# zhaotudou/HeteroFusionRCNN

Measured on AMD Instinct MI355X. Metric: KITTI frames/sec RPN train step, higher is better.
Workload: dtype f32; 1 GPU; RPN train step, hf/configs/rpn_multiclass.config: PointCNN 5 xconv (K=8; 16384/4096/1024/256/64 points; C 256..1024, X-transformation, global branch) + 6 xdconv layers + fc 256/256, 3 classes, seg head, projection of the points into the image + gather of the image feature map (B,360,1200,32) + path drop 0.9/0.9 + 'concat' fusion, bin-based box head (fc 512/512, 3x76 outputs), targets + focal/softm; frames_per_gpu=8, global_batch=8, parallelism=dp1, hip_graph=True, optimizer=hf, x_branch_on_side_stream=True, scaling=strong, library_gemm_selection=library default heuristic, gradient_exchange=none (1 rank), geometry_prefetch_depth=2, geometry_prefetch_group=12

## Files before the change

### heterofusionrcnn_amd/csrc/xconv.hip

```cpp
#include "hf_common.h"

namespace hf {

template <int M>
__device__ __forceinline__ void store_m(float *base, size_t elem, const float (&v)[M])
{
    float *p = base + elem;
    if constexpr (M == 4 || M == 8) {
        if ((reinterpret_cast<uintptr_t>(base) & 15) == 0) {
#pragma unroll
            for (int q = 0; q < M / 4; ++q) reinterpret_cast<float4 *>(p)[q] = make_float4(v[4 * q], v[4 * q + 1], v[4 * q + 2], v[4 * q + 3]);
            return;
        }
    } else if constexpr (M == 2) {
        if ((reinterpret_cast<uintptr_t>(base) & 7) == 0) { *reinterpret_cast<float2 *>(p) = make_float2(v[0], v[1]); return; }
    }
#pragma unroll
    for (int m = 0; m < M; ++m) p[m] = v[m];
}
template <int M>
__device__ __forceinline__ void load_m(const float *base, size_t elem, float (&v)[M])
{
    const float *p = base + elem;
    if constexpr (M == 4 || M == 8) {
        if ((reinterpret_cast<uintptr_t>(base) & 15) == 0) {
#pragma unroll
            for (int q = 0; q < M / 4; ++q) {
                const float4 t = reinterpret_cast<const float4 *>(p)[q];
                v[4 * q] = t.x; v[4 * q + 1] = t.y; v[4 * q + 2] = t.z; v[4 * q + 3] = t.w;
            }
            return;
        }
    } else if constexpr (M == 2) {
        if ((reinterpret_cast<uintptr_t>(base) & 7) == 0) { const float2 t = *reinterpret_cast<const float2 *>(p); v[0] = t.x; v[1] = t.y; return; }
    }
#pragma unroll
    for (int m = 0; m < M; ++m) v[m] = p[m];
}


constexpr int kXcThreads = 256;

template <int K, bool TRANSPOSED>
__global__ __launch_bounds__(kXcThreads) void xconv_apply_kernel(long long rows, int c, const float *__restrict__ x,
                                                                const float *__restrict__ f, float *__restrict__ out)
{
    const int lane = threadIdx.x & 63;
    const long long wave = __builtin_amdgcn_readfirstlane(static_cast<int>(threadIdx.x >> 6)) +
                           static_cast<long long>(blockIdx.x) * (kXcThreads / 64);
    const long long nwaves = static_cast<long long>(gridDim.x) * (kXcThreads / 64);
    for (long long r = wave; r < rows; r += nwaves) {
        const float *xr = x + r * (K * K);
        float coef[K][K];
#pragma unroll
        for (int i = 0; i < K; ++i)
#pragma unroll
            for (int j = 0; j < K; ++j) coef[i][j] = TRANSPOSED ? xr[j * K + i] : xr[i * K + j];
        const float *fr = f + r * K * c;
        float *orow = out + r * K * c;
        for (int ch = lane; ch < c; ch += 64) {
            float v[K];
#pragma unroll
            for (int j = 0; j < K; ++j) v[j] = fr[static_cast<size_t>(j) * c + ch];
#pragma unroll
            for (int i = 0; i < K; ++i) {
                float acc = coef[i][0] * v[0];
#pragma unroll
                for (int j = 1; j < K; ++j) acc = acc + coef[i][j] * v[j];
                orow[static_cast<size_t>(i) * c + ch] = acc;
            }
        }
    }
}

template <int K>
__global__ __launch_bounds__(kXcThreads) void xconv_dx_kernel(long long rows, int c, const float *__restrict__ grad_out,
                                                             const float *__restrict__ f, float *__restrict__ grad_x)
{
    extern __shared__ float lds[];
    constexpr int KK = K * K, STRIDE = KK + 1;
    const int lane = threadIdx.x & 63, w = threadIdx.x >> 6;
    float *mine = lds + static_cast<size_t>(w) * 64 * STRIDE;
    const long long wave = w + static_cast<long long>(blockIdx.x) * (kXcThreads / 64);
    const long long nwaves = static_cast<long long>(gridDim.x) * (kXcThreads / 64);
    for (long long r = wave; r < rows; r += nwaves) {
        const float *gr = grad_out + r * K * c;
        const float *fr = f + r * K * c;
        float acc[K][K];
#pragma unroll
        for (int i = 0; i < K; ++i)
#pragma unroll
            for (int j = 0; j < K; ++j) acc[i][j] = 0.f;
        for (int ch = lane; ch < c; ch += 64) {
            float g[K], v[K];
#pragma unroll
            for (int j = 0; j < K; ++j) { g[j] = gr[static_cast<size_t>(j) * c + ch]; v[j] = fr[static_cast<size_t>(j) * c + ch]; }
#pragma unroll
            for (int i = 0; i < K; ++i)
#pragma unroll
                for (int j = 0; j < K; ++j) acc[i][j] = acc[i][j] + g[i] * v[j];
        }
#pragma unroll
        for (int i = 0; i < K; ++i)
#pragma unroll
            for (int j = 0; j < K; ++j) mine[lane * STRIDE + i * K + j] = acc[i][j];
        __builtin_amdgcn_fence(__ATOMIC_SEQ_CST, "wavefront");
        __builtin_amdgcn_wave_barrier();
        for (int p = lane; p < KK; p += 64) {
            float s = 0.f;
            for (int l = 0; l < 64; ++l) s = s + mine[l * STRIDE + p];
            grad_x[r * KK + p] = s;
        }
        __builtin_amdgcn_fence(__ATOMIC_SEQ_CST, "wavefront");
        __builtin_amdgcn_wave_barrier();
    }
}

template <int K, int M>
__global__ __launch_bounds__(kXcThreads) void depthwise_fwd_kernel(long long rows, int c, const float *__restrict__ x,
                                                                  const float *__restrict__ wgt, float *__restrict__ y)
{
    const long long total = rows * c;
    for (long long g = static_cast<long long>(blockIdx.x) * kXcThreads + threadIdx.x; g < total;
         g += static_cast<long long>(gridDim.x) * kXcThreads) {
        const long long r = g / c;
        const int ch = static_cast<int>(g - r * c);
        float acc[M];
#pragma unroll
        for (int m = 0; m < M; ++m) acc[m] = 0.f;
#pragma unroll
        for (int w = 0; w < K; ++w) {
            const float xv = x[(r * K + w) * c + ch];
#pragma unroll
            for (int m = 0; m < M; ++m) acc[m] = acc[m] + xv * wgt[(static_cast<size_t>(w) * c + ch) * M + m];
        }
        store_m<M>(y, static_cast<size_t>(g) * M, acc);
    }
}

template <int K, int M>
__global__ __launch_bounds__(kXcThreads) void depthwise_dx_kernel(long long rows, int c, const float *__restrict__ grad_y,
                                                                 const float *__restrict__ wgt, float *__restrict__ grad_x)
{
    const long long total = rows * c;
    for (long long g = static_cast<long long>(blockIdx.x) * kXcThreads + threadIdx.x; g < total;
         g += static_cast<long long>(gridDim.x) * kXcThreads) {
        const long long r = g / c;
        const int ch = static_cast<int>(g - r * c);
        float gy[M];
        load_m<M>(grad_y, static_cast<size_t>(g) * M, gy);
#pragma unroll
        for (int w = 0; w < K; ++w) {
            float acc = 0.f;
#pragma unroll
            for (int m = 0; m < M; ++m) acc = acc + gy[m] * wgt[(static_cast<size_t>(w) * c + ch) * M + m];
            grad_x[(r * K + w) * c + ch] = acc;
        }
    }
}

template <int K, int M, bool DX>
__global__ __launch_bounds__(kXcThreads) void depthwise_narrow_kernel(long long rows, int c, const float *__restrict__ in,
                                                                     const float *__restrict__ wgt, float *__restrict__ out)
{
    const long long tid = static_cast<long long>(blockIdx.x) * kXcThreads + threadIdx.x;
    const long long nthreads = static_cast<long long>(gridDim.x) * kXcThreads;
    const int ch = static_cast<int>(tid % c);
    float wr[K][M];
#pragma unroll
    for (int w = 0; w < K; ++w)
#pragma unroll
        for (int m = 0; m < M; ++m) wr[w][m] = wgt[(static_cast<size_t>(w) * c + ch) * M + m];
    for (long long r = tid / c; r < rows; r += nthreads / c) {
        if (!DX) {
            float acc[M];
#pragma unroll
            for (int m = 0; m < M; ++m) acc[m] = 0.f;
#pragma unroll
            for (int w = 0; w < K; ++w) {
                const float xv = in[(r * K + w) * c + ch];
#pragma unroll
                for (int m = 0; m < M; ++m) acc[m] = acc[m] + xv * wr[w][m];
            }
            store_m<M>(out, static_cast<size_t>(r * c + ch) * M, acc);
        } else {
            float gy[M];
            load_m<M>(in, static_cast<size_t>(r * c + ch) * M, gy);
#pragma unroll
            for (int w = 0; w < K; ++w) {
                float acc = 0.f;
#pragma unroll
                for (int m = 0; m < M; ++m) acc = acc + gy[m] * wr[w][m];
                out[(r * K + w) * c + ch] = acc;
            }
        }
    }
}

static int narrow_grid(long long rows, int c)
{
    int a = c, b = kXcThreads;
    while (b) { const int tmp = a % b; a = b; b = tmp; }
    const int unit = c / a;
    long long g = (rows * c + kXcThreads - 1) / kXcThreads;
    const long long cap = static_cast<long long>(kNumCU) * 8;
    if (g > cap) g = cap;
    g = (g + unit - 1) / unit * unit;
    return static_cast<int>(g);
}
constexpr int kNarrowMaxC = 64;

template <int K, int M>
__global__ __launch_bounds__(kXcThreads) void depthwise_dw_kernel(long long rows, int c, int rows_per_chunk,
                                                                 const float *__restrict__ x, const float *__restrict__ grad_y,
                                                                 float *__restrict__ grad_w, float *__restrict__ partial)
{
    extern __shared__ float red[];
    const int cw = c < kXcThreads ? c : kXcThreads, nrs = kXcThreads / cw;
    const int t = static_cast<int>(threadIdx.x);
    const int cl = t % cw, ch = blockIdx.x * cw + cl, rs = t / cw;
    const bool live = ch < c && rs < nrs;
    if (nrs > 1) {
        for (int i = t; i < K * M * cw; i += kXcThreads) red[i] = 0.f;
        __syncthreads();
    }
    const long long r0 = static_cast<long long>(blockIdx.y) * rows_per_chunk + rs;
    const long long r1 = static_cast<long long>(blockIdx.y + 1) * rows_per_chunk < rows ? static_cast<long long>(blockIdx.y + 1) * rows_per_chunk : rows;
    float acc[K][M];
#pragma unroll
    for (int w = 0; w < K; ++w)
#pragma unroll
        for (int m = 0; m < M; ++m) acc[w][m] = 0.f;
    if (live) {
        for (long long r = r0; r < r1; r += nrs) {
            float gy[M];
            load_m<M>(grad_y, static_cast<size_t>(r * c + ch) * M, gy);
#pragma unroll
            for (int w = 0; w < K; ++w) {
                const float xv = x[(r * K + w) * c + ch];
#pragma unroll
                for (int m = 0; m < M; ++m) acc[w][m] = acc[w][m] + xv * gy[m];
            }
        }
    }
    float *mine = partial ? partial + static_cast<size_t>(blockIdx.y) * K * c * M : nullptr;
    if (nrs == 1) {
        if (live) {
#pragma unroll
            for (int w = 0; w < K; ++w)
#pragma unroll
                for (int m = 0; m < M; ++m) {
                    const size_t e = (static_cast<size_t>(w) * c + ch) * M + m;
                    if (mine) mine[e] = acc[w][m];
                    else atomicAdd(&grad_w[e], acc[w][m]);
                }
        }
        return;
    }
    const bool shuffle = (cw & (cw - 1)) == 0 && cw <= 32;
    if (shuffle) {
        const int lane = t & 63, wave = t >> 6;
        __syncthreads();
#pragma unroll
        for (int w = 0; w < K; ++w)
#pragma unroll
            for (int m = 0; m < M; ++m) {
                float v = live ? acc[w][m] : 0.f;
                for (int off = cw; off < 64; off <<= 1) v += __shfl_xor(v, off);
                if (lane < cw) red[(wave * K * M + w * M + m) * cw + lane] = v;
            }
        __syncthreads();
        for (int i = t; i < K * M * cw; i += kXcThreads) {
            float v = red[i];
#pragma unroll
            for (int wv = 1; wv < kXcThreads / 64; ++wv) v += red[wv * K * M * cw + i];
            const int wm = i / cw, c2 = blockIdx.x * cw + i % cw;
            if (c2 < c) {
                const size_t e = (static_cast<size_t>(wm / M) * c + c2) * M + wm % M;
                if (mine) mine[e] = v;
                else atomicAdd(&grad_w[e], v);
            }
        }
        return;
    }
    if (live) {
#pragma unroll
        for (int w = 0; w < K; ++w)
#pragma unroll
            for (int m = 0; m < M; ++m) atomicAdd(&red[(w * M + m) * cw + cl], acc[w][m]);
    }
    __syncthreads();
    for (int i = t; i < K * M * cw; i += kXcThreads) {
        const int wm = i / cw, c2 = blockIdx.x * cw + i % cw;
        if (c2 < c) {
            const size_t e = (static_cast<size_t>(wm / M) * c + c2) * M + wm % M;
            if (mine) mine[e] = red[i];
            else atomicAdd(&grad_w[e], red[i]);
        }
    }
}

struct XcSource {
    const float *base;
    long long stride;
    bool gathered;
};

__device__ __forceinline__ XcSource xc_source(int ch, int c, int c0, const float *f, const float *fts, const int *idx)
{
    XcSource s;
    if (idx == nullptr) { s.base = f + ch; s.stride = c; s.gathered = false; }
    else if (ch - (ch & 63) < c0) { s.base = f + ch; s.stride = c0; s.gathered = false; }
    else { s.base = fts + (ch - c0); s.stride = c - c0; s.gathered = true; }
    return s;
}

template <int K, int M, bool GATHER>
__global__ __launch_bounds__(kXcThreads) void xconv_dw_fwd_kernel(long long rows, int c, int c0, int rows_per_block,
                                                                 const float *__restrict__ x, const float *__restrict__ f,
                                                                 const float *__restrict__ fts, const int *__restrict__ idx, int n_src,
                                                                 int rows_per_cloud, const float *__restrict__ wd, float *__restrict__ out)
{
    const int lane = threadIdx.x & 63, wave = __builtin_amdgcn_readfirstlane(static_cast<int>(threadIdx.x >> 6));
    const int ch = blockIdx.y * 64 + lane;
    const bool live = ch < c;
    const XcSource src = xc_source(live ? ch : blockIdx.y * 64, c, c0, f, fts, GATHER ? idx : nullptr);
    float w[K][M];
#pragma unroll
    for (int k = 0; k < K; ++k)
#pragma unroll
        for (int m = 0; m < M; ++m) w[k][m] = live ? wd[(static_cast<size_t>(k) * c + ch) * M + m] : 0.f;
    const long long r0 = static_cast<long long>(blockIdx.x) * rows_per_block;
    const long long r1 = r0 + rows_per_block < rows ? r0 + rows_per_block : rows;
    for (long long r = r0 + wave; r < r1; r += kXcThreads / 64) {
        const float *xr = x + r * (K * K);
        float fv[K];
        const long long tbase = (GATHER && src.gathered) ? static_cast<long long>(static_cast<unsigned>(r) / static_cast<unsigned>(rows_per_cloud)) * n_src : 0;
#pragma unroll
        for (int j = 0; j < K; ++j) {
            const long long srow = (GATHER && src.gathered) ? tbase + idx[r * K + j] : r * K + j;
            fv[j] = live ? src.base[srow * src.stride] : 0.f;
        }
        float o[M];
#pragma unroll
        for (int m = 0; m < M; ++m) o[m] = 0.f;
#pragma unroll
        for (int k = 0; k < K; ++k) {
            float t = xr[k * K] * fv[0];
#pragma unroll
            for (int j = 1; j < K; ++j) t = t + xr[k * K + j] * fv[j];
#pragma unroll
            for (int m = 0; m < M; ++m) o[m] = o[m] + t * w[k][m];
        }
        if (live) store_m<M>(out, static_cast<size_t>(r * c + ch) * M, o);
    }
}

template <int K, int M, bool GATHER>
__global__ __launch_bounds__(kXcThreads) void xconv_dw_bwd_fw_kernel(long long rows, int c, int c0, int rows_per_block,
                                                                    const float *__restrict__ x, const float *__restrict__ f,
                                                                    const float *__restrict__ fts, const int *__restrict__ idx, int n_src,
                                                                    int rows_per_cloud, const float *__restrict__ wd,
                                                                    const float *__restrict__ grad_out, float *__restrict__ grad_f,
                                                                    float *__restrict__ grad_gathered, float *__restrict__ grad_wd,
                                                                    float *__restrict__ wd_partial)
{
    const int lane = threadIdx.x & 63, wave = __builtin_amdgcn_readfirstlane(static_cast<int>(threadIdx.x >> 6));
    const int ch = blockIdx.y * 64 + lane;
    const bool live = ch < c;
    const XcSource src = xc_source(live ? ch : blockIdx.y * 64, c, c0, f, fts, GATHER ? idx : nullptr);
    if (GATHER && src.gathered && !grad_wd && !grad_gathered) return;
    float w[K][M], gw[K][M];
#pragma unroll
    for (int k = 0; k < K; ++k)
#pragma unroll
        for (int m = 0; m < M; ++m) { w[k][m] = live ? wd[(static_cast<size_t>(k) * c + ch) * M + m] : 0.f; gw[k][m] = 0.f; }
    const long long r0 = static_cast<long long>(blockIdx.x) * rows_per_block;
    const long long r1 = r0 + rows_per_block < rows ? r0 + rows_per_block : rows;
    for (long long r = r0 + wave; r < r1; r += kXcThreads / 64) {
        const float *xr = x + r * (K * K);
        float fv[K], g[M], gfx[K];
        const long long tbase = (GATHER && src.gathered) ? static_cast<long long>(static_cast<unsigned>(r) / static_cast<unsigned>(rows_per_cloud)) * n_src : 0;
#pragma unroll
        for (int j = 0; j < K; ++j) {
            const long long srow = (GATHER && src.gathered) ? tbase + idx[r * K + j] : r * K + j;
            fv[j] = live ? src.base[srow * src.stride] : 0.f;
        }
        load_m<M>(grad_out, static_cast<size_t>(r * c + (live ? ch : 0)) * M, g);
        if (!live) {
#pragma unroll
            for (int m = 0; m < M; ++m) g[m] = 0.f;
        }
#pragma unroll
        for (int k = 0; k < K; ++k) {
            float a = 0.f;
#pragma unroll
            for (int m = 0; m < M; ++m) a = a + g[m] * w[k][m];
            gfx[k] = a;
            float t = xr[k * K] * fv[0];
#pragma unroll
            for (int j = 1; j < K; ++j) t = t + xr[k * K + j] * fv[j];
#pragma unroll
            for (int m = 0; m < M; ++m) gw[k][m] = gw[k][m] + t * g[m];
        }
        float *gdst = (GATHER && src.gathered) ? (grad_gathered ? grad_gathered + (ch - c0) : nullptr) : (grad_f ? grad_f + ch : nullptr);
        if (live && gdst) {
#pragma unroll
            for (int j = 0; j < K; ++j) {
                float a = xr[j] * gfx[0];
#pragma unroll
                for (int k = 1; k < K; ++k) a = a + xr[k * K + j] * gfx[k];
                gdst[(r * K + j) * src.stride] = a;
            }
        }
    }
    if (grad_wd) {
        __shared__ float red[K * M][64];
        for (int i = threadIdx.x; i < K * M * 64; i += kXcThreads) (&red[0][0])[i] = 0.f;
        __syncthreads();
        if (live) {
#pragma unroll
            for (int k = 0; k < K; ++k)
#pragma unroll
                for (int m = 0; m < M; ++m) atomicAdd(&red[k * M + m][lane], gw[k][m]);
        }
        __syncthreads();
        float *mine = wd_partial ? wd_partial + static_cast<size_t>(blockIdx.x) * K * c * M : nullptr;
        for (int i = threadIdx.x; i < K * M * 64; i += kXcThreads) {
            const int km = i >> 6, c2 = blockIdx.y * 64 + (i & 63);
            if (c2 < c) {
                const size_t e = (static_cast<size_t>(km / M) * c + c2) * M + km % M;
                if (mine) mine[e] = red[km][i & 63];
                else atomicAdd(&grad_wd[e], red[km][i & 63]);
            }
        }
    }
}

template <int K, int M, bool GATHER>
__global__ __launch_bounds__(kXcThreads) void xconv_dw_bwd_x_kernel(long long rows, int c, int c0, const float *__restrict__ f,
                                                                   const float *__restrict__ fts, const int *__restrict__ idx, int n_src,
                                                                   int rows_per_cloud, const float *__restrict__ wd,
                                                                   const float *__restrict__ grad_out, float *__restrict__ grad_x)
{
    extern __shared__ float lds[];
    constexpr int KK = K * K, STRIDE = KK + 1, QUADS = 16;
    const int lane = threadIdx.x & 63, w = threadIdx.x >> 6;
    float *mine = lds + static_cast<size_t>(w) * QUADS * STRIDE;
    const long long wave = w + static_cast<long long>(blockIdx.x) * (kXcThreads / 64);
    const long long nwaves = static_cast<long long>(gridDim.x) * (kXcThreads / 64);
    const int c1 = c - c0;
    for (long long r = wave; r < rows; r += nwaves) {
        float acc[K][K];
#pragma unroll
        for (int i = 0; i < K; ++i)
#pragma unroll
            for (int j = 0; j < K; ++j) acc[i][j] = 0.f;
        long long trow[K];
        if constexpr (GATHER) {
            const long long tbase = static_cast<long long>(static_cast<unsigned>(r) / static_cast<unsigned>(rows_per_cloud)) * n_src;
#pragma unroll
            for (int j = 0; j < K; ++j) trow[j] = tbase + idx[r * K + j];
        }
        for (int ch = lane; ch < c; ch += 64) {
            float fv[K], g[M];
            if constexpr (GATHER) {
                const bool gathered = ch >= c0;
                const float *base = gathered ? fts + (ch - c0) : f + ch;
                const long long stride = gathered ? c1 : c0;
#pragma unroll
                for (int j = 0; j < K; ++j) fv[j] = base[(gathered ? trow[j] : r * K + j) * stride];
            } else {
#pragma unroll
                for (int j = 0; j < K; ++j) fv[j] = f[(r * K + j) * c + ch];
            }
            load_m<M>(grad_out, static_cast<size_t>(r * c + ch) * M, g);
#pragma unroll
            for (int k = 0; k < K; ++k) {
                float a = 0.f;
#pragma unroll
                for (int m = 0; m < M; ++m) a = a + g[m] * wd[(static_cast<size_t>(k) * c + ch) * M + m];
#pragma unroll
                for (int j = 0; j < K; ++j) acc[k][j] = acc[k][j] + a * fv[j];
            }
        }
#pragma unroll
        for (int i = 0; i < K; ++i)
#pragma unroll
            for (int j = 0; j < K; ++j) {
                float v = acc[i][j];
                v = v + __int_as_float(__builtin_amdgcn_mov_dpp(__float_as_int(v), 0xb1, 0xf, 0xf, true));
                v = v + __int_as_float(__builtin_amdgcn_mov_dpp(__float_as_int(v), 0x4e, 0xf, 0xf, true));
                if ((lane & 3) == 0) mine[(lane >> 2) * STRIDE + i * K + j] = v;
            }
        __builtin_amdgcn_fence(__ATOMIC_SEQ_CST, "wavefront");
        __builtin_amdgcn_wave_barrier();
        for (int p = lane; p < KK; p += 64) {
            float s = 0.f;
#pragma unroll
            for (int l = 0; l < QUADS; ++l) s = s + mine[l * STRIDE + p];
            grad_x[r * KK + p] = s;
        }
        __builtin_amdgcn_fence(__ATOMIC_SEQ_CST, "wavefront");
        __builtin_amdgcn_wave_barrier();
    }
}

template <int K, int M>
__global__ __launch_bounds__(kXcThreads) void xconv_dw_bwd_fts_kernel(long long src_rows, int n_src, long long rows_per_cloud,
                                                                     int c, int c0, int rows_per_block,
                                                                     const float *__restrict__ x, const float *__restrict__ wd,
                                                                     const float *__restrict__ grad_out,
                                                                     const int *__restrict__ offsets, const int *__restrict__ entries,
                                                                     float *__restrict__ grad_fts)
{
    const int lane = threadIdx.x & 63, wave = __builtin_amdgcn_readfirstlane(static_cast<int>(threadIdx.x >> 6));
    const int c1 = c - c0, cf = blockIdx.y * 64 + lane, ch = c0 + cf;
    const bool live = cf < c1;
    float w[K][M];
#pragma unroll
    for (int k = 0; k < K; ++k)
#pragma unroll
        for (int m = 0; m < M; ++m) w[k][m] = live ? wd[(static_cast<size_t>(k) * c + ch) * M + m] : 0.f;
    const long long s0 = static_cast<long long>(blockIdx.x) * rows_per_block;
    const long long s1 = s0 + rows_per_block < src_rows ? s0 + rows_per_block : src_rows;
    long long bb = s0 / n_src;
    for (long long s = s0 + wave; s < s1; s += kXcThreads / 64) {
        while (s >= (bb + 1) * n_src) ++bb;
        const int pt = static_cast<int>(s - bb * n_src);
        const int *off = offsets + bb * (n_src + 1);
        const int *ent = entries + bb * rows_per_cloud * K;
        const int lo = off[pt], hi = off[pt + 1];
        float acc = 0.f;
        for (int e = lo; e < hi; e += 4) {
            float a4[4];
#pragma unroll
            for (int u = 0; u < 4; ++u) {
                const bool valid = e + u < hi;
                const int slot = ent[valid ? e + u : lo];
                const long long r = bb * rows_per_cloud + slot / K;
                const int j = slot % K;
                const float *xr = x + r * (K * K);
                float g[M], gfx[K];
                load_m<M>(grad_out, static_cast<size_t>(r * c + (live ? ch : 0)) * M, g);
                if (!live) {
#pragma unroll
                    for (int m = 0; m < M; ++m) g[m] = 0.f;
                }
#pragma unroll
                for (int k = 0; k < K; ++k) {
                    float a = 0.f;
#pragma unroll
                    for (int m = 0; m < M; ++m) a = a + g[m] * w[k][m];
                    gfx[k] = a;
                }
                float a = xr[j] * gfx[0];
#pragma unroll
                for (int k = 1; k < K; ++k) a = a + xr[k * K + j] * gfx[k];
                a4[u] = valid ? a : 0.f;
            }
#pragma unroll
            for (int u = 0; u < 4; ++u) acc += a4[u];
        }
        if (live) grad_fts[s * c1 + cf] = acc;
    }
}

static int grid_for(long long items, int per_block)
{
    const long long blocks = (items + per_block - 1) / per_block;
    return static_cast<int>(blocks < 1 ? 1 : (blocks > 8 * kNumCU ? 8 * kNumCU : blocks));
}

template <int K>
static int launch_apply(long long rows, int c, const float *x, const float *f, float *out, bool transposed, hipStream_t st)
{
    const int grid = grid_for(rows, kXcThreads / 64);
    if (transposed) hipLaunchKernelGGL((xconv_apply_kernel<K, true>), dim3(grid), dim3(kXcThreads), 0, st, rows, c, x, f, out);
    else hipLaunchKernelGGL((xconv_apply_kernel<K, false>), dim3(grid), dim3(kXcThreads), 0, st, rows, c, x, f, out);
    return launch_status();
}

template <int K>
static int launch_dx(long long rows, int c, const float *grad_out, const float *f, float *grad_x, hipStream_t st)
{
    const size_t lds = sizeof(float) * (kXcThreads / 64) * 64 * (K * K + 1);
    const int lrc = ensure_dynamic_lds(reinterpret_cast<const void *>(&xconv_dx_kernel<K>), lds);
    if (lrc != HF_OK) return lrc;
    hipLaunchKernelGGL((xconv_dx_kernel<K>), dim3(grid_for(rows, kXcThreads / 64)), dim3(kXcThreads), lds, st, rows, c, grad_out, f,
                       grad_x);
    return launch_status();
}

}

using namespace hf;

HF_API int hf_xconv_apply(long long rows, int k, int c, const float *x, const float *f, float *out, hf_stream_t stream)
{
    if (rows < 0 || c <= 0 || !x || !f || !out) return HF_EINVAL;
    if (rows == 0) return HF_OK;
    switch (k) {
    case 4: return launch_apply<4>(rows, c, x, f, out, false, as_stream(stream));
    case 8: return launch_apply<8>(rows, c, x, f, out, false, as_stream(stream));
    default: return HF_EINVAL;
    }
}

HF_API int hf_xconv_apply_grad(long long rows, int k, int c, const float *x, const float *f, const float *grad_out,
                               float *grad_x, float *grad_f, hf_stream_t stream)
{
    if (rows < 0 || c <= 0 || !x || !f || !grad_out || (!grad_x && !grad_f)) return HF_EINVAL;
    if (rows == 0) return HF_OK;
    hipStream_t st = as_stream(stream);
    int rc = HF_OK;
#define HF_XC_CASE(KK)                                                                                                 \
    case KK:                                                                                                           \
        if (grad_f) rc = launch_apply<KK>(rows, c, x, grad_out, grad_f, true, st);                                     \
        if (rc == HF_OK && grad_x) rc = launch_dx<KK>(rows, c, grad_out, f, grad_x, st);                               \
        return rc;
    switch (k) {
        HF_XC_CASE(4)
        HF_XC_CASE(8)
    default: return HF_EINVAL;
    }
#undef HF_XC_CASE
}

#define HF_DW_DISPATCH(CALL)                                                                                           \
    if (k == 8 && m == 1) { CALL(8, 1) } else if (k == 8 && m == 2) { CALL(8, 2) } else if (k == 8 && m == 3) { CALL(8, 3) }      \
    else if (k == 8 && m == 4) { CALL(8, 4) } else if (k == 8 && m == 8) { CALL(8, 8) }                                 \
    else if (k == 4 && m == 1) { CALL(4, 1) } else if (k == 4 && m == 4) { CALL(4, 4) }                                 \
    else return HF_EINVAL;

HF_API int hf_depthwise_k(long long rows, int k, int c, int m, const float *x, const float *w, float *y, hf_stream_t stream)
{
    if (rows < 0 || c <= 0 || !x || !w || !y) return HF_EINVAL;
    if (rows == 0) return HF_OK;
    if (c <= kNarrowMaxC && k * m <= 64) {
        const int ng = narrow_grid(rows, c);
#define HF_DW_NFWD(KK, MM) hipLaunchKernelGGL((depthwise_narrow_kernel<KK, MM, false>), dim3(ng), dim3(kXcThreads), 0, as_stream(stream), rows, c, x, w, y);
        HF_DW_DISPATCH(HF_DW_NFWD)
#undef HF_DW_NFWD
        return launch_status();
    }
    const int grid = grid_for(rows * c, kXcThreads);
#define HF_DW_FWD(KK, MM) hipLaunchKernelGGL((depthwise_fwd_kernel<KK, MM>), dim3(grid), dim3(kXcThreads), 0, as_stream(stream), rows, c, x, w, y);
    HF_DW_DISPATCH(HF_DW_FWD)
#undef HF_DW_FWD
    return launch_status();
}

static void dw_chunks(long long rows, int c, int &cblocks, int &rows_per_chunk, unsigned &nchunks)
{
    cblocks = c < kXcThreads ? 1 : div_up(c, kXcThreads);
    long long chunks = (2 * kNumCU + cblocks - 1) / cblocks;
    if (chunks > (rows + 63) / 64) chunks = (rows + 63) / 64;
    if (chunks < 1) chunks = 1;
    if (chunks > rows) chunks = rows;
    if (chunks > 65535) chunks = 65535;
    rows_per_chunk = static_cast<int>((rows + chunks - 1) / chunks);
    nchunks = static_cast<unsigned>((rows + rows_per_chunk - 1) / rows_per_chunk);
}

HF_API size_t hf_depthwise_k_grad_workspace(long long rows, int k, int c, int m)
{
    if (rows <= 0 || k <= 0 || c <= 0 || m <= 0) return 0;
    int cblocks, rpc;
    unsigned nchunks;
    dw_chunks(rows, c, cblocks, rpc, nchunks);
    return sizeof(float) * static_cast<size_t>(nchunks) * k * c * m;
}

static int depthwise_k_grad_impl(long long rows, int k, int c, int m, const float *x, const float *w, const float *grad_y,
                                 float *grad_x, float *grad_w, float *partial, hipStream_t st)
{
    if (grad_w && (!partial || rows == 0)) {
        const int rc = hip_status(hipMemsetAsync(grad_w, 0, sizeof(float) * static_cast<size_t>(k) * c * m, st));
        if (rc != HF_OK) return rc;
    }
    if (rows == 0) return HF_OK;
    if (grad_x && c <= kNarrowMaxC && k * m <= 64) {
        const int ng = narrow_grid(rows, c);
#define HF_DW_NDX(KK, MM) hipLaunchKernelGGL((depthwise_narrow_kernel<KK, MM, true>), dim3(ng), dim3(kXcThreads), 0, st, rows, c, grad_y, w, grad_x);
        HF_DW_DISPATCH(HF_DW_NDX)
#undef HF_DW_NDX
        const int rc = launch_status();
        if (rc != HF_OK) return rc;
    } else if (grad_x) {
        const int grid = grid_for(rows * c, kXcThreads);
#define HF_DW_DX(KK, MM) hipLaunchKernelGGL((depthwise_dx_kernel<KK, MM>), dim3(grid), dim3(kXcThreads), 0, st, rows, c, grad_y, w, grad_x);
        HF_DW_DISPATCH(HF_DW_DX)
#undef HF_DW_DX
        const int rc = launch_status();
        if (rc != HF_OK) return rc;
    }
    if (grad_w) {
        int cblocks, rows_per_chunk;
        unsigned nchunks;
        dw_chunks(rows, c, cblocks, rows_per_chunk, nchunks);
        const size_t lds = c <= kXcThreads / 2 ? sizeof(float) * static_cast<size_t>(k) * m * c * (((c & (c - 1)) == 0 && c <= 32) ? kXcThreads / 64 : 1) : 0;
        if (lds > 48 * 1024) return HF_EINVAL;
        const dim3 grid(cblocks, nchunks);
#define HF_DW_DW(KK, MM) hipLaunchKernelGGL((depthwise_dw_kernel<KK, MM>), grid, dim3(kXcThreads), lds, st, rows, c, rows_per_chunk, x, grad_y, grad_w, partial);
        HF_DW_DISPATCH(HF_DW_DW)
#undef HF_DW_DW
        if (partial) launch_partial_reduce(k * c * m, static_cast<int>(nchunks), partial, grad_w, st);
        return launch_status();
    }
    return HF_OK;
}

HF_API int hf_depthwise_k_grad(long long rows, int k, int c, int m, const float *x, const float *w, const float *grad_y,
                               float *grad_x, float *grad_w, hf_stream_t stream)
{
    if (rows < 0 || c <= 0 || !x || !w || !grad_y || (!grad_x && !grad_w)) return HF_EINVAL;
    return depthwise_k_grad_impl(rows, k, c, m, x, w, grad_y, grad_x, grad_w, nullptr, as_stream(stream));
}

HF_API int hf_depthwise_k_grad_ws(long long rows, int k, int c, int m, const float *x, const float *w, const float *grad_y,
                                  float *grad_x, float *grad_w, void *workspace, size_t workspace_bytes, hf_stream_t stream)
{
    if (rows < 0 || c <= 0 || !x || !w || !grad_y || (!grad_x && !grad_w)) return HF_EINVAL;
    if (grad_w && rows > 0 && (!workspace || workspace_bytes < hf_depthwise_k_grad_workspace(rows, k, c, m))) return HF_EWORKSPACE;
    return depthwise_k_grad_impl(rows, k, c, m, x, w, grad_y, grad_x, grad_w, grad_w ? static_cast<float *>(workspace) : nullptr,
                                 as_stream(stream));
}

#define HF_XDW_DISPATCH(CALL)                                                                                          \
    if (k == 8 && m == 1) { CALL(8, 1) } else if (k == 8 && m == 2) { CALL(8, 2) } else if (k == 8 && m == 3) { CALL(8, 3) }      \
    else if (k == 8 && m == 4) { CALL(8, 4) }                                                                          \
    else if (k == 4 && m == 1) { CALL(4, 1) } else if (k == 4 && m == 4) { CALL(4, 4) }    \
    else if (k == 12 && m == 1) { CALL(12, 1) } else if (k == 12 && m == 2) { CALL(12, 2) }                             \
    else return HF_EINVAL;

static void xdw_grid(long long rows, int c, dim3 &grid, int &rows_per_block, int blocks_per_cu = 8)
{
    const int cchunks = div_up(c, 64);
    long long rchunks = (blocks_per_cu * kNumCU + cchunks - 1) / cchunks;
    if (rchunks > (rows + 3) / 4) rchunks = (rows + 3) / 4;
    if (rchunks < 1) rchunks = 1;
    rows_per_block = static_cast<int>((rows + rchunks - 1) / rchunks);
    grid = dim3(static_cast<unsigned>((rows + rows_per_block - 1) / rows_per_block), cchunks);
}

static int xdw_forward(long long rows, int k, int c, int c0, int m, const float *x, const float *f, const float *fts, const int *idx,
                       int n_src, int rows_per_cloud, const float *wd, float *out, hipStream_t st)
{
    dim3 grid;
    int rpb;
    xdw_grid(rows, c, grid, rpb);
#define HF_XDW_FWD(KK, MM)                                                                                             \
    if (idx) hipLaunchKernelGGL((xconv_dw_fwd_kernel<KK, MM, true>), grid, dim3(kXcThreads), 0, st, rows, c, c0, rpb, x, f, fts, idx, n_src, rows_per_cloud, wd, out); \
    else hipLaunchKernelGGL((xconv_dw_fwd_kernel<KK, MM, false>), grid, dim3(kXcThreads), 0, st, rows, c, c0, rpb, x, f, fts, idx, n_src, rows_per_cloud, wd, out);
    HF_XDW_DISPATCH(HF_XDW_FWD)
#undef HF_XDW_FWD
    return launch_status();
}

static void xdw_bwd_grid(long long rows, int c, dim3 &grid, int &rpb)
{
    xdw_grid(rows, c, grid, rpb, 4);
    if (rpb < 32 && rows > 32) { rpb = 32; grid.x = static_cast<unsigned>((rows + rpb - 1) / rpb); }
}

static int xdw_backward(long long rows, int k, int c, int c0, int m, const float *x, const float *f, const float *fts, const int *idx,
                        int n_src, int rows_per_cloud, const float *wd, const float *grad_out, float *grad_x, float *grad_f, float *grad_gathered,
                        float *grad_wd, hipStream_t st, float *wd_partial = nullptr)
{
    if (grad_wd && (!wd_partial || rows == 0)) {
        const int rc = hip_status(hipMemsetAsync(grad_wd, 0, sizeof(float) * static_cast<size_t>(k) * c * m, st));
        if (rc != HF_OK) return rc;
    }
    if (rows == 0) return HF_OK;
    if (!grad_wd) wd_partial = nullptr;
    if (grad_f || grad_wd || grad_gathered) {
        dim3 grid;
        int rpb;
        xdw_bwd_grid(rows, c, grid, rpb);
#define HF_XDW_BFW(KK, MM)                                                                                             \
        if (idx) hipLaunchKernelGGL((xconv_dw_bwd_fw_kernel<KK, MM, true>), grid, dim3(kXcThreads), 0, st, rows, c, c0, rpb, x, f, fts, idx, n_src, rows_per_cloud, wd, grad_out, grad_f, grad_gathered, grad_wd, wd_partial); \
        else hipLaunchKernelGGL((xconv_dw_bwd_fw_kernel<KK, MM, false>), grid, dim3(kXcThreads), 0, st, rows, c, c0, rpb, x, f, fts, idx, n_src, rows_per_cloud, wd, grad_out, grad_f, grad_gathered, grad_wd, wd_partial);
        HF_XDW_DISPATCH(HF_XDW_BFW)
#undef HF_XDW_BFW
        if (wd_partial) launch_partial_reduce(k * c * m, static_cast<int>(grid.x), wd_partial, grad_wd, st);
        const int rc = launch_status();
        if (rc != HF_OK) return rc;
    }
    if (grad_x) {
        const size_t lds = sizeof(float) * (kXcThreads / 64) * 16 * (static_cast<size_t>(k) * k + 1);
#define HF_XDW_BX(KK, MM)                                                                                              \
        if (idx) hipLaunchKernelGGL((xconv_dw_bwd_x_kernel<KK, MM, true>), dim3(grid_for(rows, kXcThreads / 64)), dim3(kXcThreads), lds, st, rows, c, c0, f, fts, idx, n_src, rows_per_cloud, wd, grad_out, grad_x); \
        else hipLaunchKernelGGL((xconv_dw_bwd_x_kernel<KK, MM, false>), dim3(grid_for(rows, kXcThreads / 64)), dim3(kXcThreads), lds, st, rows, c, c0, f, fts, idx, n_src, rows_per_cloud, wd, grad_out, grad_x);
        HF_XDW_DISPATCH(HF_XDW_BX)
#undef HF_XDW_BX
        return launch_status();
    }
    return HF_OK;
}

HF_API int hf_xconv_depthwise(long long rows, int k, int c, int m, const float *x, const float *f, const float *wd, float *out,
                              hf_stream_t stream)
{
    if (rows < 0 || c <= 0 || !x || !f || !wd || !out) return HF_EINVAL;
    if (rows == 0) return HF_OK;
    return xdw_forward(rows, k, c, c, m, x, f, nullptr, nullptr, 0, 1, wd, out, as_stream(stream));
}

HF_API int hf_xconv_depthwise_grad(long long rows, int k, int c, int m, const float *x, const float *f, const float *wd,
                                   const float *grad_out, float *grad_x, float *grad_f, float *grad_wd, hf_stream_t stream)
{
    if (rows < 0 || c <= 0 || !x || !f || !wd || !grad_out || (!grad_x && !grad_f && !grad_wd)) return HF_EINVAL;
    return xdw_backward(rows, k, c, c, m, x, f, nullptr, nullptr, 0, 1, wd, grad_out, grad_x, grad_f, nullptr, grad_wd, as_stream(stream));
}

HF_API int hf_xconv_depthwise_gather(int b, int n_src, int rows_per_cloud, int k, int c0, int c1, int m, const float *x,
                                     const float *f_delta, const float *fts, const int *idx, const float *wd, float *out,
                                     hf_stream_t stream)
{
    if (b < 0 || n_src <= 0 || rows_per_cloud < 0 || c0 <= 0 || c0 % 64 != 0 || c1 <= 0) return HF_EINVAL;
    const long long rows = static_cast<long long>(b) * rows_per_cloud;
    if (rows == 0) return HF_OK;
    if (rows > 0x7fffffffll || !x || !f_delta || !fts || !idx || !wd || !out) return HF_EINVAL;
    return xdw_forward(rows, k, c0 + c1, c0, m, x, f_delta, fts, idx, n_src, rows_per_cloud, wd, out, as_stream(stream));
}

static size_t xdw_gathered_bytes(int b, int rows_per_cloud, int k, int c1)
{
    return (sizeof(float) * static_cast<size_t>(b) * rows_per_cloud * k * c1 + 255) & ~static_cast<size_t>(255);
}

HF_API size_t hf_xconv_depthwise_gather_grad_workspace(int b, int rows_per_cloud, int k, int c0, int c1, int m)
{
    if (b <= 0 || rows_per_cloud <= 0 || k <= 0 || c0 <= 0 || c1 <= 0 || m <= 0) return 0;
    dim3 grid;
    int rpb;
    xdw_bwd_grid(static_cast<long long>(b) * rows_per_cloud, c0 + c1, grid, rpb);
    return xdw_gathered_bytes(b, rows_per_cloud, k, c1) + sizeof(float) * static_cast<size_t>(grid.x) * k * (c0 + c1) * m;
}

HF_API int hf_xconv_depthwise_gather_grad(int b, int n_src, int rows_per_cloud, int k, int c0, int c1, int m, const float *x,
                                          const float *f_delta, const float *fts, const int *idx, const float *wd,
                                          const float *grad_out, const int *offsets, const int *entries, float *grad_x,
                                          float *grad_f_delta, float *grad_fts, float *grad_wd, void *workspace,
                                          size_t workspace_bytes, hf_stream_t stream)
{
    if (b < 0 || n_src <= 0 || rows_per_cloud < 0 || c0 <= 0 || c0 % 64 != 0 || c1 <= 0 || !x || !f_delta || !fts || !idx || !wd ||
        !grad_out || static_cast<long long>(b) * rows_per_cloud > 0x7fffffffll ||
        (!grad_x && !grad_f_delta && !grad_fts && !grad_wd))
        return HF_EINVAL;
    if (grad_fts && (!offsets || !entries)) return HF_EINVAL;
    if (workspace && workspace_bytes < hf_xconv_depthwise_gather_grad_workspace(b, rows_per_cloud, k, c0, c1, m)) return HF_EWORKSPACE;
    hipStream_t st = as_stream(stream);
    const long long rows = static_cast<long long>(b) * rows_per_cloud;
    const int c = c0 + c1;
    float *gathered = (grad_fts && workspace) ? static_cast<float *>(workspace) : nullptr;
    float *wd_partial = workspace ? reinterpret_cast<float *>(static_cast<unsigned char *>(workspace) + xdw_gathered_bytes(b, rows_per_cloud, k, c1)) : nullptr;
    if (grad_x || grad_f_delta || grad_wd || gathered) {
        const int rc = xdw_backward(rows, k, c, c0, m, x, f_delta, fts, idx, n_src, rows_per_cloud, wd, grad_out, grad_x, grad_f_delta, gathered,
                                    grad_wd, st, wd_partial);
        if (rc != HF_OK) return rc;
    }
    if (grad_fts) {
        const long long src_rows = static_cast<long long>(b) * n_src;
        if (src_rows == 0) return HF_OK;
        if (rows == 0) return hip_status(hipMemsetAsync(grad_fts, 0, sizeof(float) * static_cast<size_t>(src_rows) * c1, st));
        if (gathered) return hf_group_point_grad_gather(b, n_src, c1, rows_per_cloud, k, c1, 0, gathered, offsets, entries, grad_fts, stream);
        dim3 grid;
        int rpb;
        xdw_grid(src_rows, c1, grid, rpb);
#define HF_XDW_FTS(KK, MM) hipLaunchKernelGGL((xconv_dw_bwd_fts_kernel<KK, MM>), grid, dim3(kXcThreads), 0, st, src_rows, n_src, static_cast<long long>(rows_per_cloud), c, c0, rpb, x, wd, grad_out, offsets, entries, grad_fts);
        HF_XDW_DISPATCH(HF_XDW_FTS)
#undef HF_XDW_FTS
        return launch_status();
    }
    return HF_OK;
}
```

Measured before the change: 294.4 frames/s.

## Process channel pairs and staged X rows in depthwise xconv forward kernel

Rewrites the depthwise X-conv forward kernel so each lane handles two adjacent channels with float2 loads and stores, halving the channel-chunk grid dimension. Each wave processes two rows per iteration, loading the K×K X-transform rows coalesced across lanes and staging them through LDS instead of every lane reading them redundantly. The per-cloud gather base is tracked incrementally rather than divided per row, and 32-bit offsets are used. This adds a guard that rejects inputs whose offsets exceed 32 bits, and a scalar fallback for odd channel counts or misaligned pointers.

```diff
diff --git a/heterofusionrcnn_amd/csrc/xconv.hip b/heterofusionrcnn_amd/csrc/xconv.hip
--- a/heterofusionrcnn_amd/csrc/xconv.hip
+++ b/heterofusionrcnn_amd/csrc/xconv.hip
@@ -1,4 +1,6 @@
 #include "hf_common.h"
+
+#include <initializer_list>
 
 namespace hf {
 
@@ -300,6 +302,169 @@
     }
 }
 
+typedef float f2 __attribute__((ext_vector_type(2)));
+
+struct XcPair {
+    const float *base;
+    unsigned hi;
+    bool gathered, live, hi_live;
+};
+
+__device__ __forceinline__ XcPair xc_pair(int ch, int c, int c0, const float *f, const float *fts, bool gather)
+{
+    XcPair s;
+    s.live = ch < c;
+    s.hi_live = ch + 1 < c;
+    const int cc = s.live ? ch : (c - 1) & ~1;
+    s.hi = s.hi_live ? 1u : 0u;
+    s.gathered = gather && cc >= c0;
+    s.base = s.gathered ? fts + (cc - c0) : f + cc;
+    return s;
+}
+
+template <bool V2>
+__device__ __forceinline__ f2 ld_pair(const float *p, unsigned hi)
+{
+    if constexpr (V2) return *reinterpret_cast<const f2 *>(p);
+    else return f2{p[0], p[hi]};
+}
+
+template <int M, bool V2>
+__device__ __forceinline__ void st_pair_m(float *p, bool hi_live, const f2 (&v)[M])
+{
+    if constexpr (V2) {
+#pragma unroll
+        for (int q = 0; q < M; ++q) {
+            const int e0 = 2 * q, e1 = 2 * q + 1;
+            reinterpret_cast<f2 *>(p)[q] = f2{e0 < M ? v[e0].x : v[e0 - M].y, e1 < M ? v[e1].x : v[e1 - M].y};
+        }
+    } else {
+#pragma unroll
+        for (int m = 0; m < M; ++m) p[m] = v[m].x;
+        if (hi_live) {
+#pragma unroll
+            for (int m = 0; m < M; ++m) p[M + m] = v[m].y;
+        }
+    }
+}
+
+constexpr int kXcRows = 2;
+
+struct XcCloud {
+    long long next;
+    unsigned tbase;
+};
+
+__device__ __forceinline__ unsigned xc_tbase(XcCloud &cl, long long r, int rows_per_cloud, int n_src)
+{
+    while (r >= cl.next) { cl.next += rows_per_cloud; cl.tbase += static_cast<unsigned>(n_src); }
+    return cl.tbase;
+}
+
+__device__ __forceinline__ XcCloud xc_cloud(long long r, int rows_per_cloud, int n_src)
+{
+    const long long b = r / rows_per_cloud;
+    return XcCloud{(b + 1) * rows_per_cloud, static_cast<unsigned>(b * n_src)};
+}
+
+template <int K, bool GATHER, bool V2>
+__device__ __forceinline__ void xc_gather_row(const XcPair &s, long long r, unsigned tbase, const int *__restrict__ idx,
+                                              unsigned lstride, unsigned c1, f2 (&fv)[K])
+{
+    const unsigned rk = static_cast<unsigned>(r) * K;
+#pragma unroll
+    for (int j = 0; j < K; ++j) {
+        const unsigned lo = (rk + j) * lstride;
+        unsigned off = lo;
+        if constexpr (GATHER) {
+            const unsigned go = (tbase + static_cast<unsigned>(idx[rk + j])) * c1;
+            off = s.gathered ? go : lo;
+        }
+        fv[j] = ld_pair<V2>(s.base + off, s.hi);
+    }
+}
+
+template <int K>
+struct XcXRows {
+    static constexpr int KK = K * K, Q = (KK + 63) / 64;
+    float v[kXcRows][Q];
+    __device__ __forceinline__ void load(const float *__restrict__ x, const long long (&rr)[kXcRows], int lane)
+    {
+#pragma unroll
+        for (int i = 0; i < kXcRows; ++i)
+#pragma unroll
+            for (int q = 0; q < Q; ++q) {
+                const int p = lane + 64 * q;
+                v[i][q] = x[rr[i] * KK + (p < KK ? p : KK - 1)];
+            }
+    }
+    __device__ __forceinline__ void stage(float (*xs)[KK], int lane) const
+    {
+        __builtin_amdgcn_fence(__ATOMIC_SEQ_CST, "wavefront");
+        __builtin_amdgcn_wave_barrier();
+#pragma unroll
+        for (int i = 0; i < kXcRows; ++i)
+#pragma unroll
+            for (int q = 0; q < Q; ++q)
+                if (lane + 64 * q < KK) xs[i][lane + 64 * q] = v[i][q];
+        __builtin_amdgcn_fence(__ATOMIC_SEQ_CST, "wavefront");
+        __builtin_amdgcn_wave_barrier();
+    }
+};
+
+template <int K, int M, bool GATHER, bool V2>
+__global__ __launch_bounds__(kXcThreads) void xconv_dw_fwd_kernel(long long rows, int c, int c0, int rows_per_block,
+                                                                 const float *__restrict__ x, const float *__restrict__ f,
+                                                                 const float *__restrict__ fts, const int *__restrict__ idx, int n_src,
+                                                                 int rows_per_cloud, const float *__restrict__ wd, float *__restrict__ out)
+{
+    const int lane = threadIdx.x & 63, wave = __builtin_amdgcn_readfirstlane(static_cast<int>(threadIdx.x >> 6));
+    const int ch = blockIdx.y * 128 + 2 * lane;
+    const XcPair src = xc_pair(ch, c, c0, f, fts, GATHER);
+    const int cw = src.live ? ch : (c - 1) & ~1;
+    f2 w[K][M];
+#pragma unroll
+    for (int k = 0; k < K; ++k)
+#pragma unroll
+        for (int m = 0; m < M; ++m) w[k][m] = f2{wd[(static_cast<size_t>(k) * c + cw) * M + m], wd[(static_cast<size_t>(k) * c + cw + src.hi) * M + m]};
+    const unsigned lstride = GATHER ? c0 : c, c1 = c - c0;
+    const long long r0 = static_cast<long long>(blockIdx.x) * rows_per_block;
+    const long long r1 = r0 + rows_per_block < rows ? r0 + rows_per_block : rows;
+    __shared__ float xs[kXcThreads / 64][kXcRows][K * K];
+    XcCloud cl = xc_cloud(r0, rows_per_cloud, n_src);
+    for (long long rb = r0 + wave; rb < r1; rb += 4 * kXcRows) {
+        f2 fv[kXcRows][K];
+        long long rr[kXcRows];
+#pragma unroll
+        for (int i = 0; i < kXcRows; ++i) rr[i] = rb + 4 * i < r1 ? rb + 4 * i : r1 - 1;
+        XcXRows<K> xrow;
+        xrow.load(x, rr, lane);
+#pragma unroll
+        for (int i = 0; i < kXcRows; ++i) {
+            const unsigned tb = GATHER ? xc_tbase(cl, rr[i], rows_per_cloud, n_src) : 0u;
+            xc_gather_row<K, GATHER, V2>(src, rr[i], tb, idx, lstride, c1, fv[i]);
+        }
+        xrow.stage(xs[wave], lane);
+#pragma unroll
+        for (int i = 0; i < kXcRows; ++i) {
+            if (rb + 4 * i >= r1) break;
+            const float *xr = xs[wave][i];
+            f2 o[M];
+#pragma unroll
+            for (int m = 0; m < M; ++m) o[m] = f2{0.f, 0.f};
+#pragma unroll
+            for (int k = 0; k < K; ++k) {
+                f2 t = xr[k * K] * fv[i][0];
+#pragma unroll
+                for (int j = 1; j < K; ++j) t = t + xr[k * K + j] * fv[i][j];
+#pragma unroll
+                for (int m = 0; m < M; ++m) o[m] = o[m] + t * w[k][m];
+            }
+            if (src.live) st_pair_m<M, V2>(out + static_cast<size_t>(rr[i] * c + ch) * M, src.hi_live, o);
+        }
+    }
+}
+
 struct XcSource {
     const float *base;
     long long stride;
@@ -313,47 +478,6 @@
     else if (ch - (ch & 63) < c0) { s.base = f + ch; s.stride = c0; s.gathered = false; }
     else { s.base = fts + (ch - c0); s.stride = c - c0; s.gathered = true; }
     return s;
-}
-
-template <int K, int M, bool GATHER>
-__global__ __launch_bounds__(kXcThreads) void xconv_dw_fwd_kernel(long long rows, int c, int c0, int rows_per_block,
-                                                                 const float *__restrict__ x, const float *__restrict__ f,
-                                                                 const float *__restrict__ fts, const int *__restrict__ idx, int n_src,
-                                                                 int rows_per_cloud, const float *__restrict__ wd, float *__restrict__ out)
-{
-    const int lane = threadIdx.x & 63, wave = __builtin_amdgcn_readfirstlane(static_cast<int>(threadIdx.x >> 6));
-    const int ch = blockIdx.y * 64 + lane;
-    const bool live = ch < c;
-    const XcSource src = xc_source(live ? ch : blockIdx.y * 64, c, c0, f, fts, GATHER ? idx : nullptr);
-    float w[K][M];
-#pragma unroll
-    for (int k = 0; k < K; ++k)
-#pragma unroll
-        for (int m = 0; m < M; ++m) w[k][m] = live ? wd[(static_cast<size_t>(k) * c + ch) * M + m] : 0.f;
-    const long long r0 = static_cast<long long>(blockIdx.x) * rows_per_block;
-    const long long r1 = r0 + rows_per_block < rows ? r0 + rows_per_block : rows;
-    for (long long r = r0 + wave; r < r1; r += kXcThreads / 64) {
-        const float *xr = x + r * (K * K);
-        float fv[K];
-        const long long tbase = (GATHER && src.gathered) ? static_cast<long long>(static_cast<unsigned>(r) / static_cast<unsigned>(rows_per_cloud)) * n_src : 0;
-#pragma unroll
-        for (int j = 0; j < K; ++j) {
-            const long long srow = (GATHER && src.gathered) ? tbase + idx[r * K + j] : r * K + j;
-            fv[j] = live ? src.base[srow * src.stride] : 0.f;
-        }
-        float o[M];
-#pragma unroll
-        for (int m = 0; m < M; ++m) o[m] = 0.f;
-#pragma unroll
-        for (int k = 0; k < K; ++k) {
-            float t = xr[k * K] * fv[0];
-#pragma unroll
-            for (int j = 1; j < K; ++j) t = t + xr[k * K + j] * fv[j];
-#pragma unroll
-            for (int m = 0; m < M; ++m) o[m] = o[m] + t * w[k][m];
-        }
-        if (live) store_m<M>(out, static_cast<size_t>(r * c + ch) * M, o);
-    }
 }
 
 template <int K, int M, bool GATHER>
@@ -734,9 +858,9 @@
     else if (k == 12 && m == 1) { CALL(12, 1) } else if (k == 12 && m == 2) { CALL(12, 2) }                             \
     else return HF_EINVAL;
 
-static void xdw_grid(long long rows, int c, dim3 &grid, int &rows_per_block, int blocks_per_cu = 8)
-{
-    const int cchunks = div_up(c, 64);
+static void xdw_grid(long long rows, int c, dim3 &grid, int &rows_per_block, int blocks_per_cu = 8, int chunk = 64)
+{
+    const int cchunks = div_up(c, chunk);
     long long rchunks = (blocks_per_cu * kNumCU + cchunks - 1) / cchunks;
     if (rchunks > (rows + 3) / 4) rchunks = (rows + 3) / 4;
     if (rchunks < 1) rchunks = 1;
@@ -744,17 +868,36 @@
     grid = dim3(static_cast<unsigned>((rows + rows_per_block - 1) / rows_per_block), cchunks);
 }
 
+static bool xdw_offsets_fit(long long rows, int k, int c, long long src_rows)
+{
+    return rows * k * static_cast<long long>(c) < (1ll << 32) && src_rows * static_cast<long long>(c) < (1ll << 32);
+}
+
+static bool xdw_v2(int c, std::initializer_list<const void *> ptrs)
+{
+    if (c & 1) return false;
+    for (const void *p : ptrs)
+        if (reinterpret_cast<uintptr_t>(p) & 7) return false;
+    return true;
+}
+
+static void xdw_pair_grid(long long rows, int c, dim3 &grid, int &rpb, int blocks_per_cu) { xdw_grid(rows, c, grid, rpb, blocks_per_cu, 128); }
+
 static int xdw_forward(long long rows, int k, int c, int c0, int m, const float *x, const float *f, const float *fts, const int *idx,
                        int n_src, int rows_per_cloud, const float *wd, float *out, hipStream_t st)
 {
+    if (!xdw_offsets_fit(rows, k, c, idx ? static_cast<long long>(rows / rows_per_cloud) * n_src : 0)) return HF_EINVAL;
     dim3 grid;
     int rpb;
-    xdw_grid(rows, c, grid, rpb);
-#define HF_XDW_FWD(KK, MM)                                                                                             \
-    if (idx) hipLaunchKernelGGL((xconv_dw_fwd_kernel<KK, MM, true>), grid, dim3(kXcThreads), 0, st, rows, c, c0, rpb, x, f, fts, idx, n_src, rows_per_cloud, wd, out); \
-    else hipLaunchKernelGGL((xconv_dw_fwd_kernel<KK, MM, false>), grid, dim3(kXcThreads), 0, st, rows, c, c0, rpb, x, f, fts, idx, n_src, rows_per_cloud, wd, out);
+    xdw_pair_grid(rows, c, grid, rpb, 8);
+    const bool v2 = xdw_v2(c, {f, fts, out});
+#define HF_XDW_FWD_V(KK, MM, V)                                                                                        \
+    if (idx) hipLaunchKernelGGL((xconv_dw_fwd_kernel<KK, MM, true, V>), grid, dim3(kXcThreads), 0, st, rows, c, c0, rpb, x, f, fts, idx, n_src, rows_per_cloud, wd, out); \
+    else hipLaunchKernelGGL((xconv_dw_fwd_kernel<KK, MM, false, V>), grid, dim3(kXcThreads), 0, st, rows, c, c0, rpb, x, f, fts, idx, n_src, rows_per_cloud, wd, out);
+#define HF_XDW_FWD(KK, MM) if (v2) { HF_XDW_FWD_V(KK, MM, true) } else { HF_XDW_FWD_V(KK, MM, false) }
     HF_XDW_DISPATCH(HF_XDW_FWD)
 #undef HF_XDW_FWD
+#undef HF_XDW_FWD_V
     return launch_status();
 }
 
```

New measurement: 299.7 frames/s, median of 6. 1.8% higher.
